# kspalaiologos/modern-rzip

Hardware: AMD Instinct MI355X
Metric: rzip-stage GiB/s (mrzip -n) (higher is better)
Workload: dtype u8; 1 GPU; tar-64G: rzip stage of mrzip -L7 on a 64 GiB synthetic tar (60 % text members, 25 % noise, 15 % exact duplicates, 512-byte aligned; BASELINE configs[2], the largest single-GPU configuration), one chunk per GPU, input resident in HBM; level=7, chunk_bytes_per_gpu=68719476736, streams=1, mode=streams

## Files before the change

### modern-rzip_amd/csrc/mrz_seq_deep.hip

```cpp
#ifndef MRZ_DEEP_WAVES
#define MRZ_DEEP_WAVES 8
#endif
#define MRZ_SEQ_WAVES MRZ_DEEP_WAVES
#include "mrz_seq_common.h"
#include <cstddef>

#ifndef MRZ_DEEP_LANES
#define MRZ_DEEP_LANES 256
#endif
#ifndef MRZ_DEEP_GROUP
#define MRZ_DEEP_GROUP 8
#endif
#define MRZ_DEEP_THREADS (64 * MRZ_DEEP_WAVES)
#ifdef __HIP_DEVICE_COMPILE__
#define MRZ_DEEP_WAIT() asm volatile("s_waitcnt vmcnt(0)" ::: "memory")
#else
#define MRZ_DEEP_WAIT() ((void)0)
#endif
#ifdef MRZ_SEQ_PROFILE
#define DPROF_T0() int64_t dprof_t0 = (int64_t)__builtin_amdgcn_s_memtime()
#define DPROF_T0R() dprof_t0 = (int64_t)__builtin_amdgcn_s_memtime()
#define DPROF_ADD(acc)                                               \
    do {                                                             \
        const int64_t now__ = (int64_t)__builtin_amdgcn_s_memtime(); \
// ... 100 lines not shown
    return (unsigned)fwd | (lngf << 7) | ((unsigned)rawb << 8);
}

__device__ __forceinline__ int mrz_deep_pair_eval(unsigned raw, int64_t q, int64_t op, int64_t floor_p) {
    if (op >= q) return 0;
    const int fwd = (int)(raw & 127u), rawb = (int)((raw >> 8) & 127u);
    int64_t maxb = q - floor_p;
    if (op < maxb) maxb = op;
    if (maxb < 0) maxb = 0;
    const int edge = op < 64 ? (int)(op >> 4) : 4;
    if (((raw >> 7) & 1u) || (rawb == 64 && maxb > 64) || (edge < 4 && rawb >= 16 * edge && maxb > 16 * edge)) return 1;
    const int rv = rawb < maxb ? rawb : (int)maxb;
    return fwd + rv >= MRZ_MIN_MATCH ? 1 : 0;
}

__device__ __forceinline__ unsigned mrz_deep_hs(unsigned x) { return (x * 2654435761u) >> (32 - 11); }
static_assert(MRZ_DEEP_MAP == 2048, "mrz_deep_hs gives 11 bits");
static_assert(MRZ_DEEP_LANES * 4 <= MRZ_DEEP_MAP * 3 / 4 || MRZ_DEEP_LANES <= 256, "the maps hold a batch's writes");

__device__ static void mrz_deep_smap_put(mrz_deep_lds *S, int slot, int lane_no) {
    const unsigned key = (unsigned)slot + 1u;
    unsigned i = mrz_deep_hs(key);
    for (int n = 0; n < MRZ_DEEP_MAP; n++) {
        const unsigned k = atomicCAS(&S->smap_key[i], 0u, key);
        if (k == 0u || k == key) {
            atomicMin(&S->smap_lane[i], lane_no);
            return;
        }
        i = (i + 1) & (MRZ_DEEP_MAP - 1);
    }
}
__device__ static int mrz_deep_smap_get(const mrz_deep_lds *S, int slot) {
    if (slot < 0) return 0x7fffffff;
    const unsigned key = (unsigned)slot + 1u;
    unsigned i = mrz_deep_hs(key);
    for (int n = 0; n < MRZ_DEEP_MAP; n++) {
        const unsigned k = S->smap_key[i];
        if (k == 0u) return 0x7fffffff;
        if (k == key) return S->smap_lane[i];
        i = (i + 1) & (MRZ_DEEP_MAP - 1);
    }
    return 0;
}
__device__ static void mrz_deep_tmap_put(mrz_deep_lds *S, int64_t tag, int lane_no) {
    if (tag == 0) return;
    const unsigned long long key = (unsigned long long)tag;
    unsigned i = mrz_deep_hs((unsigned)(key ^ (key >> 23)));
    for (int n = 0; n < MRZ_DEEP_MAP; n++) {
        const unsigned long long k = atomicCAS(&S->tmap_key[i], 0ull, key);
        if (k == 0ull || k == key) {
            atomicMin(&S->tmap_lane[i], lane_no);
            return;
        }
        i = (i + 1) & (MRZ_DEEP_MAP - 1);
    }
}
__device__ static int mrz_deep_tmap_get(const mrz_deep_lds *S, int64_t tag) {
    if (tag == 0) return 0x7fffffff;
    const unsigned long long key = (unsigned long long)tag;
    unsigned i = mrz_deep_hs((unsigned)(key ^ (key >> 23)));
    for (int n = 0; n < MRZ_DEEP_MAP; n++) {
        const unsigned long long k = S->tmap_key[i];
        if (k == 0ull) return 0x7fffffff;
        if (k == key) return S->tmap_lane[i];
        i = (i + 1) & (MRZ_DEEP_MAP - 1);
    }
    return 0;
}

__device__ __forceinline__ int mrz_deep_cw_slot(const mrz_deep_lds *S, int64_t cw_base, int r) {
    int lo = 0, hi = MRZ_DEEP_CW_WORDS - 1;
#pragma unroll
    for (int it = 0; it < 5; it++) {
        const int mid = (lo + hi + 1) >> 1;
        if (S->cwcum[mid] <= r)
            lo = mid;
        else
            hi = mid - 1;
    }
    return (int)(cw_base + lo * 64 + mrz_select64(S->cw[lo], r - S->cwcum[lo]));
}
static_assert(MRZ_DEEP_CW_WORDS == 32, "mrz_deep_cw_slot searches 32 words in 5 steps");

__device__ static void mrz_deep_scan(const mrz_cfg &C, mrz_deep_lds *S, int i, int64_t better, int64_t tag_mask,
                                     int64_t clean_ptr, int xw_n, int lane, int from = 0) {
    const mrz_slot *tab = C.tab;
    const uint8_t *__restrict__ buf = C.buf;
    const int smask = (int)C.slot_mask;
    const int max_chain = (int)C.max_chain;
    const int64_t q = mrz_uni64(S->R.q[i]), t = mrz_uni64(S->R.t[i]);
    const bool ins = (t & tag_mask) == tag_mask;
    const int my_rank = mrz_ones_rank(t);
    const int h = (int)(t & C.slot_mask);
    int fe = -1, w = -1, kind = ins ? -1 : MRZ_DK_NONE;
    int nsame = 0, round = 0;
    bool cplx = false;
    int64_t occ_t = 0, occ_off = 0, old_t = 0;
    bool cont = false, insert_kept = false, fe2 = false;
    int nsame0 = 0;
    int alt_w = -1, alt_kind = MRZ_DK_NONE, alt_st = 0, alt_round = 0;
    int64_t alt_old_t = 0;
    if (from > 0) {
        const int f0 = mrz_uni((int)S->R.flags[i]), k0 = mrz_uni((int)S->R.kind[i]);
        const int ns0 = mrz_uni((int)S->R.nsame[i]);
        if (!(f0 & MRZ_DF_CPLX) && k0 != MRZ_DK_EVICT && k0 != MRZ_DK_DISPLACE && from <= ((mrz_uni(S->R.fe[i]) - h) & smask)) {
            cont = true;
            const bool before = lane < ns0 && ((S->R.same_slot[i][lane < MRZ_SMAX ? lane : 0] - h) & smask) < from;
            nsame0 = nsame = __popcll(__ballot(before));
            if (ins && (k0 == MRZ_DK_EMPTY || k0 == MRZ_DK_OVER) && ((mrz_uni(S->R.w[i]) - h) & smask) < from) {
                insert_kept = true;
                kind = k0;
                w = mrz_uni(S->R.w[i]);
                old_t = mrz_uni64(S->R.old_t[i]);
            } else
                round = nsame;
        }
    }
    const int start = cont ? from : 0;
    const int max_groups = (int)((C.nslots + 64 * MRZ_DEEP_GROUP - 1) / (64 * MRZ_DEEP_GROUP)) + 1;
    for (int grp = 0; fe < 0; grp++) {
        if (grp >= max_groups) {
            cplx = true;
            fe = h;
            break;
        }
        mrz_slot e[MRZ_DEEP_GROUP];
        const int s0 = h + start + grp * (64 * MRZ_DEEP_GROUP) + lane;
#pragma unroll
        for (int g = 0; g < MRZ_DEEP_GROUP; g++) e[g] = tab[(s0 + g * 64) & smask];
#pragma unroll
        for (int g = 0; g < MRZ_DEEP_GROUP; g++) {
            if (fe >= 0) continue;
            const int sb = s0 - lane + g * 64;
            const bool empty = (e[g].off | e[g].t) == 0;
            const mrz_u64 m_empty = __ballot(empty);
            const int fe_idx = m_empty ? __ffsll((long long)m_empty) - 1 : 64;
            const mrz_u64 valid = mrz_low_mask(fe_idx);
            const mrz_u64 m_same = __ballot(!empty && e[g].t == t) & valid;
            mrz_u64 m_due = 0, m_low = 0;
            if (kind == -1 || alt_st == 1) {
                m_due = __ballot(!empty && (e[g].t & better) != better) & valid;
                m_low = __ballot(!empty && mrz_ones_rank(e[g].t) < my_rank) & valid & ~m_due;
            }
            int alt_from = 0;
            if (kind == -1) {
                const mrz_u64 m_stop = m_due | m_low;
                const int ks = m_stop ? __ffsll((long long)m_stop) - 1 : 64;
                const int nq = __popcll(m_same & mrz_low_mask(ks));
                if (round + nq >= max_chain) {
                    kind = MRZ_DK_EVICT;
                } else {
                    round += nq;
                    if (ks < 64) {
                        w = (sb + ks) & smask;
                        if ((m_due >> ks) & 1) {
                            kind = MRZ_DK_OVER;
                            old_t = mrz_bcast64(e[g].t, ks);
                            alt_st = 1;
                            alt_from = ks + 1;
                            alt_round = round;
                        } else {
                            kind = MRZ_DK_DISPLACE;
                            occ_t = mrz_bcast64(e[g].t, ks);
                            occ_off = mrz_bcast64(e[g].off, ks);
                        }
                    } else if (fe_idx < 64) {
                        w = (sb + fe_idx) & smask;
                        kind = MRZ_DK_EMPTY;
                        if (fe_idx < 63 && ((m_empty >> (fe_idx + 1)) & 1)) {
                            alt_w = (sb + fe_idx + 1) & smask;
                            alt_kind = MRZ_DK_EMPTY;
                        }
                        alt_st = 2;
                    }
                }
            }
            if (alt_st == 1 && alt_from < 64) {
                const mrz_u64 beyond = ~mrz_low_mask(alt_from);
                const mrz_u64 m_stop2 = (m_due | m_low) & beyond;
                const int ks2 = m_stop2 ? __ffsll((long long)m_stop2) - 1 : 64;
                const int nq2 = __popcll(m_same & beyond & mrz_low_mask(ks2));
                if (alt_round + nq2 >= max_chain)
                    alt_st = 2;
                else {
                    alt_round += nq2;
                    if (ks2 < 64) {
                        if ((m_due >> ks2) & 1) {
                            alt_w = (sb + ks2) & smask;
                            alt_kind = MRZ_DK_OVER;
                            alt_old_t = mrz_bcast64(e[g].t, ks2);
                        }
                        alt_st = 2;
                    } else if (fe_idx < 64) {
                        alt_w = (sb + fe_idx) & smask;
                        alt_kind = MRZ_DK_EMPTY;
                        alt_st = 2;
                    }
                }
            }
            if (m_same) {
                if ((m_same >> lane) & 1) {
                    const int k = nsame + __popcll(m_same & mrz_low_mask(lane));
                    if (k < MRZ_SMAX) {
                        S->R.same_slot[i][k] = (sb + lane) & smask;
                        S->R.same_off[i][k] = e[g].off;
                    }
                }
                nsame += __popcll(m_same);
            }
            if (fe_idx < 64) {
                fe = (sb + fe_idx) & smask;
                fe2 = fe_idx < 63 && ((m_empty >> (fe_idx + 1)) & 1);
            }
        }
    }
    if (nsame > MRZ_SMAX) cplx = true;
    if (kind == MRZ_DK_EVICT && max_chain > MRZ_SMAX) cplx = true;
    int h2 = 0, w2 = -1, kind2 = MRZ_DK_NONE;
    int64_t old_t2 = 0;
    if (kind == MRZ_DK_DISPLACE && !cplx) {
        const int rank2 = mrz_ones_rank(occ_t);
        h2 = (int)(occ_t & C.slot_mask);
        int round2 = 0;
        bool done = false;
        for (int grp = 0; !done; grp++) {
            if (grp >= max_groups) {
                cplx = true;
                break;
            }
            mrz_slot e[MRZ_DEEP_GROUP];
            const int s0 = h2 + grp * (64 * MRZ_DEEP_GROUP) + lane;
#pragma unroll
            for (int g = 0; g < MRZ_DEEP_GROUP; g++) e[g] = tab[(s0 + g * 64) & smask];
#pragma unroll
            for (int g = 0; g < MRZ_DEEP_GROUP; g++) {
                if (done) continue;
                const int sb = s0 - lane + g * 64;
                const bool empty = (e[g].off | e[g].t) == 0;
                const bool due = !empty && (e[g].t & better) != better;
                const bool low = !empty && !due && mrz_ones_rank(e[g].t) < rank2;
                const mrz_u64 m_empty = __ballot(empty), m_due = __ballot(due), m_low = __ballot(low);
                const mrz_u64 m_stop = m_empty | m_due | m_low;
                const int ks = m_stop ? __ffsll((long long)m_stop) - 1 : 64;
                const int nq = __popcll(__ballot(!empty && !due && !low && e[g].t == occ_t) & mrz_low_mask(ks));
                if (round2 + nq >= max_chain) {
                    cplx = true;
                    done = true;
                } else if (ks < 64) {
                    if ((m_low >> ks) & 1)
                        cplx = true;
                    else {
                        w2 = (sb + ks) & smask;
                        kind2 = ((m_empty >> ks) & 1) ? MRZ_DK_EMPTY : MRZ_DK_OVER;
                        if (kind2 == MRZ_DK_OVER) old_t2 = mrz_bcast64(e[g].t, ks);
                    }
                    done = true;
                } else
                    round2 += nq;
            }
        }
    }
    const int ns = nsame < MRZ_SMAX ? nsame : MRZ_SMAX;
    if (ns > nsame0) {
        MRZ_WAVE_SYNC();
        if (lane >= nsame0 && lane < ns) S->R.raw[i][lane] = (unsigned short)mrz_deep_probe_raw(buf, q, S->R.same_off[i][lane], C.end);
    }
    if (lane == 0) {
        S->R.h[i] = h;
        S->R.fe[i] = fe;
        S->R.w[i] = w;
        S->R.kind[i] = (unsigned char)(kind < 0 ? MRZ_DK_NONE : kind);
        S->R.h2[i] = h2;
        S->R.w2[i] = w2;
        S->R.kind2[i] = (unsigned char)kind2;
        S->R.occ_t[i] = occ_t;
        S->R.occ_off[i] = occ_off;
        S->R.old_t[i] = old_t;
        S->R.old_t2[i] = old_t2;
        S->R.alt_w[i] = (cplx || kind == MRZ_DK_DISPLACE || kind == MRZ_DK_EVICT || insert_kept) ? -1 : alt_w;
        S->R.alt_kind[i] = (unsigned char)alt_kind;
        S->R.alt_old_t[i] = alt_old_t;
        S->R.nsame[i] = (unsigned char)ns;
        S->R.flags[i] = (unsigned char)((ins ? MRZ_DF_INS : 0) | (cplx ? MRZ_DF_CPLX : 0) | (fe2 ? MRZ_DF_FE2 : 0));
        if (!cont) {
            S->R.cp_scan[i] = clean_ptr;
            S->R.xw_seen[i] = (unsigned short)xw_n;
        }
    }
}

#ifndef MRZ_DEEP_SCANNERS
#define MRZ_DEEP_SCANNERS 63
#endif
#define MRZ_DEEP_STAMP_RETRIES (1 << 20)
#ifndef MRZ_DEEP_HELP_MIN
#define MRZ_DEEP_HELP_MIN 48
#endif

#define MRZ_DEEP_REC_HDR 5
#define MRZ_DEEP_REC_GRANULES (MRZ_DEEP_REC_HDR + MRZ_SMAX)
struct mrz_deep_rec_ent {
    int64_t same_off;
    int same_slot;
    unsigned short raw, pad;
};
struct __attribute__((aligned(16))) mrz_deep_rec {
    int64_t occ_t, occ_off;
    int64_t old_t, old_t2;
    int64_t cp_scan, alt_old_t;
    int alt_w, h, fe, w;
    int h2, w2;
    unsigned short xw_seen;
    unsigned char kind, kind2, nsame, flags, alt_kind, pad;
    mrz_deep_rec_ent ent[MRZ_SMAX];
};
static_assert(sizeof(mrz_deep_rec_ent) == 16 && sizeof(mrz_deep_rec) == 16 * MRZ_DEEP_REC_GRANULES, "records travel as 16-byte granules");
// ... 102 lines not shown
#else
struct mrz_deep_recmem {
    char *base;
};
__device__ __forceinline__ mrz_deep_recmem mrz_deep_recmem_of(mrz_deep_shared *G) {
    mrz_deep_recmem m;
    m.base = (char *)G->rec;
    return m;
}
__device__ __forceinline__ void mrz_deep_granule_store(const mrz_deep_recmem &m, unsigned off, uint4 v) {
    *(uint4 *)(m.base + off) = v;
}
__device__ __forceinline__ uint4 mrz_deep_granule_load(const mrz_deep_recmem &m, bool take, unsigned off, int soff) {
    return take ? *(const uint4 *)(m.base + off + soff) : make_uint4(0, 0, 0, 0);
}
#endif

__device__ __forceinline__ void mrz_deep_rec_send(const mrz_deep_recmem &m, const mrz_deep_lds *S, int i, int lane) {
    MRZ_WAVE_SYNC();
    const int ng = MRZ_DEEP_REC_HDR + mrz_uni((int)S->R.nsame[i]);
    if (lane < ng) mrz_deep_granule_store(m, (unsigned)(i * (int)sizeof(mrz_deep_rec) + lane * 16), mrz_deep_rec_granule(&S->R, i, lane));
}

#define MRZ_DEEP_REC_FIRST (MRZ_DEEP_REC_HDR + 1)
#define MRZ_DEEP_FETCH_PER (MRZ_DEEP_THREADS / MRZ_DEEP_REC_FIRST)
__device__ __forceinline__ void mrz_deep_recs_fetch(mrz_deep_shared *G, mrz_deep_lds *S, int nb, int nscan, int tid) {
    const mrz_deep_recmem m = mrz_deep_recmem_of(G);
    constexpr int NLD = (MRZ_DEEP_LANES + MRZ_DEEP_FETCH_PER - 1) / MRZ_DEEP_FETCH_PER;
    constexpr int CH = 5;
#ifdef __HIP_DEVICE_COMPILE__
    asm volatile("" : "+v"(tid));
#endif
    const int i0 = tid / MRZ_DEEP_REC_FIRST, g = tid - i0 * MRZ_DEEP_REC_FIRST;
    const unsigned off0 = (unsigned)(i0 * (int)sizeof(mrz_deep_rec) + g * 16);
    bool take[NLD];
#pragma unroll
    for (int j = 0; j < NLD; j++) {
        const int i = i0 + j * MRZ_DEEP_FETCH_PER;
        take[j] = i0 < MRZ_DEEP_FETCH_PER && i < nb && i % nscan != 0;
    }
    uint4 v[NLD];
#pragma unroll
    for (int j = 0; j < NLD; j++) {
        v[j] = mrz_deep_granule_load(m, take[j], off0, j * MRZ_DEEP_FETCH_PER * (int)sizeof(mrz_deep_rec));
    }
#pragma unroll
    for (int j = 0; j < NLD; j++)
        if (take[j]) mrz_deep_rec_ungranule(&S->R, i0 + j * MRZ_DEEP_FETCH_PER, g, v[j], MRZ_SMAX);
    __syncthreads();
    const int ns = (tid < nb && tid % nscan != 0) ? (int)S->R.nsame[tid] : 0;
    for (int k0 = 1; __ballot(k0 < ns) != 0; k0 += CH) {
        const unsigned offe = (unsigned)(tid * (int)sizeof(mrz_deep_rec) + (MRZ_DEEP_REC_HDR + k0) * 16);
        uint4 e[CH];
#pragma unroll
        for (int c = 0; c < CH; c++) {
            e[c] = mrz_deep_granule_load(m, k0 + c < ns, offe, c * 16);
        }
#pragma unroll
        for (int c = 0; c < CH; c++)
            if (k0 + c < ns) mrz_deep_rec_ungranule(&S->R, tid, MRZ_DEEP_REC_HDR + k0 + c, e[c], ns);
    }
}

__device__ static void mrz_deep_scan_helper(const mrz_cfg &C, mrz_deep_lds *S, mrz_deep_shared *G, int tid, int lane, int wave) {
    if (tid == 0) {
        long long spins = 0;
        unsigned long long x = 0;
        while ((x = __hip_atomic_load(&G->xcc_plus1, __ATOMIC_RELAXED, __HIP_MEMORY_SCOPE_AGENT)) == 0 &&
               !__hip_atomic_load(&G->quit, __ATOMIC_RELAXED, __HIP_MEMORY_SCOPE_AGENT) && spins++ < (1ll << 24))
            __builtin_amdgcn_s_sleep(8);
        int ticket = -1;
        if (x != 0)
            ticket = (int)__hip_atomic_fetch_add(&G->n_ok, 1ull, __ATOMIC_RELAXED, __HIP_MEMORY_SCOPE_AGENT);
        S->ctl[0] = ticket;
    }
    __syncthreads();
    const int ticket = mrz_uni(S->ctl[0]);
    if (ticket < 0 || ticket >= MRZ_DEEP_SCANNERS) return;
    const int me = ticket + 1;
    const mrz_deep_recmem recmem = mrz_deep_recmem_of(G);
    unsigned long long seen = 0;
    int retries = 0;
#ifdef MRZ_SEQ_PROFILE
    int64_t hprof[4] = {0, 0, 0, 0};
#endif
    DPROF_T0();
    while (true) {
        if (tid == 0) {
            long long spins = 0;
            unsigned long long sq = 0;
            int v = 1;
            while (true) {
                sq = __hip_atomic_load(&G->seq, __ATOMIC_RELAXED, __HIP_MEMORY_SCOPE_AGENT);
                if (sq != seen && retries == 0) break;
                if (__hip_atomic_load(&G->quit, __ATOMIC_RELAXED, __HIP_MEMORY_SCOPE_AGENT) || spins++ > MRZ_HELPER_SPIN_LIMIT) {
                    v = 0;
                    break;
                }
                if (sq != seen) break;
                __builtin_amdgcn_s_sleep(2);
            }
            DPROF_T0R();
            MRZ_DEEP_ACQUIRE();
            MRZ_DEEP_WAIT();
            S->ctl[1] = v;
            S->lead.p = (int64_t)sq;
        }
        __syncthreads();
        if (!mrz_uni(S->ctl[1])) break;
        DPROF_ADD(hprof[0]);
        const unsigned long long sq = (unsigned long long)mrz_uni64(S->lead.p);
        const uint4 sv = *(const uint4 *)&G->stamp;
        const unsigned long long job_seq = (unsigned long long)mrz_uni64((int64_t)(((unsigned long long)sv.y << 32) | sv.x));
        const int nb = mrz_uni((int)sv.z), nscan = mrz_uni((int)sv.w);
        const int xw_n = (int)G->xw_n;
        const int64_t better = G->better, tag_mask = G->tag_mask, clean_ptr = G->clean_ptr;
        if (job_seq != sq) {
            if (++retries > MRZ_DEEP_STAMP_RETRIES) break;
            __syncthreads();
            continue;
        }
        retries = 0;
        seen = sq;
        int mine_n = 0;
        if (me < nscan) {
            for (int i = me + tid * nscan; i < nb; i += nscan * MRZ_DEEP_THREADS) {
                S->R.q[i] = G->q[i];
                S->R.t[i] = G->t[i];
            }
            __syncthreads();
            DPROF_ADD(hprof[1]);
            int k = 0;
            for (int i = me; i < nb; i += nscan, k++)
                if (k % MRZ_DEEP_WAVES == wave) {
                    mrz_deep_scan(C, S, i, better, tag_mask, clean_ptr, xw_n, lane);
                    mrz_deep_rec_send(recmem, S, i, lane);
                }
            mine_n = k;
            MRZ_DEEP_WAIT();
#ifdef MRZ_SEQ_PROFILE
            __syncthreads();
            DPROF_ADD(hprof[2]);
#endif
        }
        __syncthreads();
        if (tid == 0 && mine_n) {
#ifdef MRZ_DEEP_HANDOFF_FENCED
            MRZ_DEEP_RELEASE();
            MRZ_DEEP_WAIT();
#endif
            __hip_atomic_fetch_add(&G->done, (unsigned long long)mine_n, __ATOMIC_RELAXED, __HIP_MEMORY_SCOPE_AGENT);
            DPROF_ADD(hprof[3]);
        }
    }
#ifdef MRZ_SEQ_PROFILE
    if (tid == 0 && ticket == 0)
        for (int k = 0; k < 4; k++) C.st->prof[MRZ_ST_DH_T_ACQ + k] += hprof[k];
#endif
}

__device__ static __attribute__((noinline)) bool mrz_deep_coop(const mrz_cfg &C, mrz_lead &L, mrz_coop_lds *B, int64_t t,
                                                               int lane, int64_t *stat) {
    return mrz_seq_candidate(C, L, B, t, lane, stat);
}

__device__ static __attribute__((noinline)) bool mrz_deep_candidate_rec(const mrz_cfg &C, mrz_lead &L, mrz_deep_lds *S, int i, int *xw_n, int lane,
                                              int64_t *stat) {
    mrz_coop_lds *B = &S->coop;
    const int64_t q = mrz_uni64(S->R.q[i]), t = mrz_uni64(S->R.t[i]);
    const int ns = mrz_uni((int)S->R.nsame[i]);
    const int f = mrz_uni((int)S->R.flags[i]);
    int64_t mlen = 0, m_off = 0, m_rev = 0;
    L.p = q;
    if (ns) {
        if (lane < ns) {
            const int64_t op = S->R.same_off[i][lane];
            B->same_off[lane] = op;
            int64_t ml, rv;
            bool lng;
            mrz_lane_match_len(C.buf, q, op, C.end, L.last_match, &ml, &rv, &lng);
            B->pair_res[lane] = lng ? -1 : (int)((ml << 8) | rv);
        }
        MRZ_WAVE_SYNC();
        int xh = 0, xm = 0;
        if (!mrz_resolve_entries(C, L, B, q, ns, lane, stat, &mlen, &m_off, &m_rev, &xh, &xm)) return false;
        L.tag_hits += xh;
        L.tag_misses += xm;
    }
    int nx = *xw_n;
    if (f & MRZ_DF_INS) {
        const int kind = mrz_uni((int)S->R.kind[i]);
        L.inserts++;
        L.count++;
        int ws = mrz_uni(S->R.w[i]);
        if (kind == MRZ_DK_OVER)
            L.count--;
        else if (kind == MRZ_DK_EVICT) {
            L.count--;
            ws = mrz_uni(S->R.same_slot[i][(int)L.victim_round]);
            L.victim_round = L.victim_round + 1 == C.max_chain ? 0 : L.victim_round + 1;
        } else if (kind == MRZ_DK_DISPLACE) {
            const int w2 = mrz_uni(S->R.w2[i]);
            if (mrz_uni((int)S->R.kind2[i]) == MRZ_DK_OVER) L.count--;
            if (lane == 0) {
                mrz_slot oc;
                oc.off = S->R.occ_off[i];
                oc.t = S->R.occ_t[i];
                C.tab[w2] = oc;
                S->xw_slot[nx] = w2;
            }
            nx++;
        }
        if (lane == 0) {
            mrz_slot nw;
            nw.off = q;
            nw.t = t;
            C.tab[ws] = nw;
            S->xw_slot[nx] = ws;
        }
        nx++;
        if (L.count > C.limit) {
            MRZ_DEEP_WAIT();
            mrz_cull_one(C, L, lane);
            if (lane == 0) S->xw_slot[nx] = (int)L.clean_ptr;
            nx++;
        }
    }
    *xw_n = nx;
    return mrz_select_emit(C, L, mlen, m_off, m_rev, lane);
}

__device__ __forceinline__ int mrz_deep_incl(int v, int *ws, int lane, int wave, int *total) {
    const int incl = mrz_wave_incl_sum(v, lane);
    if (lane == 63) ws[wave] = incl;
    __syncthreads();
    int add = 0, tot = 0;
#pragma unroll
    for (int w = 0; w < MRZ_DEEP_WAVES; w++) {
        const int x = ws[w];
        tot += x;
// ... 603 lines not shown
                        ST_ADD(MRZ_ST_D_COOP, 1);
                        ST_ADD(MRZ_ST_D_COOP_REC, rec ? 1 : 0);
                        const bool same_masks = L.min_mask == mm0 && L.tag_mask == tm0;
                        const int nwr = rec ? 0 : mrz_uni(S->coop.n_written);
                        const int64_t cs = rec ? -1 : mrz_uni64(S->coop.cull_slot);
                        const bool room = nx + nwr + 1 <= MRZ_DEEP_XW;
                        if (rec)
                            nx = nx_rec;
                        else if (okc && same_masks && room && !loose) {
                            if (lane < nwr) S->xw_slot[nx + lane] = (int)S->coop.pend_h[lane];
                            nx += nwr;
                            if (cs >= 0) {
                                if (lane == 0) S->xw_slot[nx] = (int)cs;
                                nx++;
                            }
                        }
                        verdict = !okc ? 3 : ((same_masks && (room || loose) && L.p >= q) ? 1 : 2);
                        if (!(loose && verdict == 1)) break;
                        int j = cl + 1;
                        while (j < nb && mrz_uni64(S->R.q[j]) <= L.p) j++;
                        if (j >= nb) break;
                        cl = j;
                    }
                    if (lane == 0) {
                        S->lead = L;
                        S->ctl[0] = verdict;
                        S->ctl[5] = nx;
                    }
                    MRZ_DEEP_WAIT();
                }
                __syncthreads();
                L = S->lead;
                xw_n = mrz_uni(S->ctl[5]);
                const int v = mrz_uni(S->ctl[0]);
                if (v == 3) ok = false;
                if (v == 2) cut = true;
                {
                    const int i = tid;
                    const int nf = mrz_deep_first(i > coop_lane && i < nb && S->R.q[i] > L.p, S->wmin3, lane, wave, tid, nb);
                    next = nf;
                }
                PROF_ADD(MRZ_ST_D_T_COOP);
            }
        }
        if (ok) {
            if (cut || L.p > mrz_uni64(S->R.q[nb - 1])) {
                int64_t pos = L.p + 1;
                if (pos < K.seg_start) pos = K.seg_start;
                ci = mrz_cand_lower_bound(K, pos, lane);
            } else
                ci += n_examined;
        }
        __syncthreads();
    }
    if (ok && ci >= K.n && L.p < lim) L.p = lim;
#ifdef MRZ_SEQ_PROFILE
    stat[MRZ_ST_D_T_TOTAL] += (int64_t)__builtin_amdgcn_s_memtime() - launch_t0;
#endif
    if (tid == 0) {
        if (G) __hip_atomic_store(&G->quit, 1ull, __ATOMIC_RELAXED, __HIP_MEMORY_SCOPE_AGENT);
#if MRZ_HELPER_WGS > 0
        if (C.gmb) mrz_g_storeu(&C.gmb->quit, 1ull);
#endif
        st->p = L.p;
        st->cur_p = L.cur_p;
        st->cur_ofs = L.cur_ofs;
        st->cur_len = L.cur_len;
        st->last_match = L.last_match;
        st->min_mask = L.min_mask;
        st->tag_mask = L.tag_mask;
        st->count = L.count;
        st->clean_ptr = L.clean_ptr;
        st->victim_round = L.victim_round;
        st->n_events = L.n_events;
        st->inserts = L.inserts;
        st->tag_hits = L.tag_hits;
        st->tag_misses = L.tag_misses;
        st->finished = L.p >= C.end ? 1 : 0;
        st->hint_positions = L.p - hint_p0;
        st->hint_events = L.n_events - hint_ev0;
        st->hint_matched = L.mbytes;
#ifdef MRZ_SEQ_STATS
        for (int k = 0; k < MRZ_ST_N; k++)
            if (k < MRZ_ST_DH_T_ACQ || k > MRZ_ST_DH_T_OUT) st->prof[k] += stat[k];
#endif
    }
}

extern "C" hipError_t mrz_launch_sequencer_deep(hipStream_t stream, const uint8_t *buf, mrz_slot *tab, const mrz_cand *cand,
                                                const int *tile_off, const mrz_u64 *bitmap, mrz_event *events,
                                                mrz_seq_state *st, void *gmailbox, int n_helpers, int xcd, void *deep_shared,
                                                int scanners) {
    mrz_seq_args a;
    a.buf = buf;
    a.tab = tab;
    a.cand = cand;
    a.tile_off = tile_off;
    a.bitmap = bitmap;
    a.events = events;
    a.st = st;
    a.gmailbox = gmailbox;
    a.xcd = xcd & 7;
    a.deep_bits = 0;
#if MRZ_HELPER_WGS == 0
    n_helpers = 0;
#endif
    if (n_helpers > MRZ_HELPER_WGS) n_helpers = MRZ_HELPER_WGS;
    if (n_helpers < 0 || !gmailbox) n_helpers = 0;
    a.n_helpers = n_helpers;
    if (gmailbox) {
        hipError_t e = hipMemsetAsync(gmailbox, 0, sizeof(mrz_gmailbox), stream);
        if (e != hipSuccess) return e;
    }
    if (scanners < 0 || !deep_shared) scanners = 0;
    if (scanners > MRZ_DEEP_SCANNERS) scanners = MRZ_DEEP_SCANNERS;
    unsigned grid = (unsigned)(1 + a.n_helpers);
    if (grid < (unsigned)(a.xcd + 1)) grid = (unsigned)(a.xcd + 1);
#ifdef MRZ_EMU_LDS_PER_BLOCK
    if (scanners > 0) {
        grid = (unsigned)(8 * scanners + a.xcd + 1);
        emu::request_coresident();
    }
#else
    if (scanners > a.n_helpers / 2) scanners = a.n_helpers / 2;
    while (scanners > 0 && grid < (unsigned)(scanners + 2)) scanners--;
#endif
    if (deep_shared) {
        hipError_t e = hipMemsetAsync(deep_shared, 0, offsetof(mrz_deep_shared, q), stream);
        if (e != hipSuccess) return e;
    }
    hipLaunchKernelGGL(mrz_seq_deep_kernel, dim3(grid), dim3(MRZ_DEEP_THREADS), 0, stream, a, (mrz_deep_shared *)deep_shared,
                       scanners);
    return hipGetLastError();
}

extern "C" size_t mrz_seq_deep_shared_size(void) { return sizeof(mrz_deep_shared); }
```

### modern-rzip_amd/csrc/mrz_seq_stats.h

```cpp
#pragma once
#include "mrz_common.h"

#define MRZ_SEQ_STATS_LIST(X) \
    X(BATCHES, "batches") X(FORMED, "formed") X(COMMITTED, "committed") X(SEGMENTS, "segments") \
    X(EMITS, "emits") X(BACKJUMP, "backjump") X(REWALK, "rewalk") X(LONGRES, "longres") X(SEQ, "seq_cands") \
    X(CUT_CPLX, "cut_cplx") X(CUT_OVERFLOW, "cut_overflow") X(SKIPOUT, "skipout") X(CONF0, "conf0") \
    X(PAIRS, "pairs") X(T_FORM, "t_form") X(T_WALK, "t_walk") X(T_CONF, "t_conf") X(T_PAIRS, "t_pairs") \
    X(T_LOOP, "t_loop") X(T_REWALK, "t_rewalk") X(T_LONG, "t_long") X(T_SEQ, "t_seq") X(FARMED, "farmed") \
    X(L_POST, "l_post") X(L_STRIPE, "l_stripe") X(L_BWD, "l_bwd") X(L_WAIT, "l_wait") X(L_ROUNDS, "l_rounds") \
    X(F_POST, "f_post") X(F_WAIT, "f_wait") X(F_FOLD, "f_fold") X(S_TAB, "s_tab") X(S_PAIR, "s_pair") \
    X(S_INS, "s_ins") X(OVL, "ovl") X(OVL_OK, "ovl_ok") X(X_WALK, "x_walk") X(X_CASC, "x_casc") \
    X(X_POOL, "x_pool") X(X_WIN, "x_win") X(X_SAME, "x_same") X(C_WIN, "c_win") X(C_EVICT, "c_evict") \
    X(C_DEEP, "c_deep") X(C_MANY, "c_many") X(C_FAIL, "c_fail") X(C_TIE, "c_tie") X(C_NW, "c_nw") \
    X(T_OVL, "t_ovl") X(H_PRE, "h_pre") X(H_CAND, "h_cand") X(H_POST, "h_post") X(T_SCAN, "t_scan") \
    X(T_FOLD, "t_fold") X(T_COMMIT, "t_commit") X(REPREP, "reprep") X(W_STALE, "w_stale") X(W_DROP, "w_drop") \
    X(RESET, "reset") X(T_TURN, "t_turn") X(T_PREP, "t_prep") X(T_PRECOMMIT, "t_precommit") X(E_MASK, "e_mask") \
    X(E_CULL, "e_cull") X(E_XW, "e_xw") X(E_INWIN, "e_inwin") X(E_WINDOW, "e_window") X(E_BULK, "e_bulk") \
    X(E_MORE, "e_more") X(T_PC_CW, "t_pc_cw") X(T_PC_LOG, "t_pc_log") X(T_PC_BEST, "t_pc_best") \
    X(T_PC_BULK, "t_pc_bulk") X(T_TURNWORK, "t_turnwork") X(T_SNAP, "t_snap") X(REBULK, "rebulk") \
     \
    X(BATCH_LANES, "batch_lanes") X(CUT_LONG, "cut_long") X(CUT_WALK, "cut_walk") \
    X(CUT_CONFLICT, "cut_conflict") X(CUT_CULL, "cut_cull") X(BATCH_EMITS, "batch_emits") \
    X(CUT_CASCADE, "cut_cascade") X(BATCH_FORMED, "batch_formed") X(T_WALK2, "t_walk2") X(T_SCANS, "t_scans") \
    X(T_CONFLICT, "t_conflict") X(T_WINDOW, "t_window") \
     \
    X(D_BATCHES, "d_batches") X(D_LANES, "d_lanes") X(D_ROUNDS, "d_rounds") X(D_RESCANNED, "d_rescanned") \
    X(D_COOP, "d_coop") X(D_T_FORM, "d_t_form") X(D_T_SCAN, "d_t_scan") X(D_T_COMMIT, "d_t_commit") \
    X(D_T_RESCAN, "d_t_rescan") X(D_T_TOTAL, "d_t_total") X(D_LAUNCHES, "d_launches") X(D_T_COOP, "d_t_coop") \
    X(D_COOP_REC, "d_coop_rec") X(D_RESOLVED, "d_resolved") X(D_S_COOP, "d_s_coop") \
    X(D_S_CONFLICT, "d_s_conflict") X(D_S_CULLED, "d_s_culled") X(D_S_NOCULL, "d_s_nocull") \
    X(D_S_STALE, "d_s_stale") X(D_C_OVER_ALT, "d_c_over_alt") X(D_C_OVER_NOALT, "d_c_over_noalt") \
    X(D_C_EMPTY, "d_c_empty") X(D_C_DISPLACE, "d_c_displace") X(D_C_OTHER, "d_c_other") \
     \
    X(D_T_POST, "d_t_post") X(D_T_OWN, "d_t_own") X(D_T_WAIT, "d_t_wait") X(D_T_COPYIN, "d_t_copyin") \
    X(DH_T_ACQ, "dh_t_acq") X(DH_T_JOB, "dh_t_job") X(DH_T_SCAN, "dh_t_scan") X(DH_T_OUT, "dh_t_out")

#define MRZ_ST_ENUM(id, name) MRZ_ST_##id,
enum { MRZ_SEQ_STATS_LIST(MRZ_ST_ENUM) MRZ_ST_N };
#undef MRZ_ST_ENUM
static_assert(MRZ_ST_N <= (int)(sizeof(((mrz_seq_state *)0)->prof) / sizeof(int64_t)), "mrz_seq_state.prof holds the counters");
```

Baseline: 6.767 GiB/s.

## Double-buffer deep-scan table loads and skip quiet groups with one ballot

The deep hash-table scan now issues the next group of slot loads before processing the current one, using a two-set register buffer and a partial vmcnt wait, so memory latency overlaps the ballot logic. It also adds a fast path that skips a whole group when no lane sees an empty, same-tag or stop-worthy entry, replacing eight rounds of ballots with one. Scalar parameters are forced uniform and loads go through global address-space byte offsets to cut address arithmetic. The cost is more vector registers, which may lower occupancy, and one extra speculative group load per scan.

```diff
diff --git a/modern-rzip_amd/csrc/mrz_seq_deep.hip b/modern-rzip_amd/csrc/mrz_seq_deep.hip
--- a/modern-rzip_amd/csrc/mrz_seq_deep.hip
+++ b/modern-rzip_amd/csrc/mrz_seq_deep.hip
@@ -206,16 +206,70 @@
 }
 static_assert(MRZ_DEEP_CW_WORDS == 32, "mrz_deep_cw_slot searches 32 words in 5 steps");
 
+#if defined(__HIP_DEVICE_COMPILE__) && !defined(MRZ_DEEP_SCAN_FLAT)
+typedef long long mrz_deep_v2l __attribute__((ext_vector_type(2)));
+typedef const __attribute__((address_space(1))) char *mrz_deep_tab;
+__device__ __forceinline__ mrz_deep_tab mrz_deep_tab_of(const mrz_slot *tab) {
+    return (mrz_deep_tab)(uintptr_t)mrz_uni64((int64_t)(uintptr_t)tab);
+}
+__device__ __forceinline__ mrz_slot mrz_deep_tab_ld(mrz_deep_tab tab, unsigned byte_off) {
+    const mrz_deep_v2l v = *(const __attribute__((address_space(1))) mrz_deep_v2l *)(tab + byte_off);
+    mrz_slot e;
+    e.off = v.x;
+    e.t = v.y;
+    return e;
+}
+#else
+typedef const mrz_slot *mrz_deep_tab;
+__device__ __forceinline__ mrz_deep_tab mrz_deep_tab_of(const mrz_slot *tab) { return tab; }
+__device__ __forceinline__ mrz_slot mrz_deep_tab_ld(mrz_deep_tab tab, unsigned byte_off) { return tab[byte_off >> 4]; }
+#endif
+#if defined(__HIP_DEVICE_COMPILE__) && !defined(MRZ_DEEP_SCAN_VECTOR_STATE)
+#define MRZ_DEEP_UNI(v) mrz_uni(v)
+#define MRZ_DEEP_UNI64(v) mrz_uni64(v)
+#else
+#define MRZ_DEEP_UNI(v) (v)
+#define MRZ_DEEP_UNI64(v) (v)
+#endif
+#ifdef __HIP_DEVICE_COMPILE__
+#define MRZ_DEEP_SCHED_FENCE() __builtin_amdgcn_sched_barrier(0)
+#else
+#define MRZ_DEEP_SCHED_FENCE() ((void)0)
+#endif
+#ifdef MRZ_SEQ_PROFILE
+#define MRZ_DSCAN_PROF_PARAM , int64_t *wprof = nullptr
+#define DSCAN_T0() int64_t dscan_t0 = wprof ? (int64_t)__builtin_amdgcn_s_memtime() : 0
+#define DSCAN_WAIT(n) asm volatile("s_waitcnt vmcnt(%0) lgkmcnt(0)" ::"n"(n) : "memory")
+#define DSCAN_ADD(k)                                                     \
+    do {                                                                 \
+        if (wprof) {                                                     \
+            const int64_t now__ = (int64_t)__builtin_amdgcn_s_memtime(); \
+            wprof[k] += now__ - dscan_t0;                                \
+            dscan_t0 = now__;                                            \
+        }                                                                \
+    } while (0)
+#else
+#define MRZ_DSCAN_PROF_PARAM
+#define DSCAN_T0()
+#define DSCAN_WAIT(n)
+#define DSCAN_ADD(k)
+#endif
 __device__ static void mrz_deep_scan(const mrz_cfg &C, mrz_deep_lds *S, int i, int64_t better, int64_t tag_mask,
-                                     int64_t clean_ptr, int xw_n, int lane, int from = 0) {
-    const mrz_slot *tab = C.tab;
+                                     int64_t clean_ptr, int xw_n, int lane, int from = 0 MRZ_DSCAN_PROF_PARAM) {
+    i = MRZ_DEEP_UNI(i);
+    from = MRZ_DEEP_UNI(from);
+    xw_n = MRZ_DEEP_UNI(xw_n);
+    better = MRZ_DEEP_UNI64(better);
+    tag_mask = MRZ_DEEP_UNI64(tag_mask);
+    clean_ptr = MRZ_DEEP_UNI64(clean_ptr);
+    const mrz_deep_tab tab = mrz_deep_tab_of(C.tab);
     const uint8_t *__restrict__ buf = C.buf;
-    const int smask = (int)C.slot_mask;
-    const int max_chain = (int)C.max_chain;
+    const int smask = MRZ_DEEP_UNI((int)C.slot_mask);
+    const int max_chain = MRZ_DEEP_UNI((int)C.max_chain);
     const int64_t q = mrz_uni64(S->R.q[i]), t = mrz_uni64(S->R.t[i]);
     const bool ins = (t & tag_mask) == tag_mask;
     const int my_rank = mrz_ones_rank(t);
-    const int h = (int)(t & C.slot_mask);
+    const int h = (int)(t & (int64_t)smask);
     int fe = -1, w = -1, kind = ins ? -1 : MRZ_DK_NONE;
     int nsame = 0, round = 0;
     bool cplx = false;
@@ -241,110 +295,157 @@
         }
     }
     const int start = cont ? from : 0;
-    const int max_groups = (int)((C.nslots + 64 * MRZ_DEEP_GROUP - 1) / (64 * MRZ_DEEP_GROUP)) + 1;
-    for (int grp = 0; fe < 0; grp++) {
+    const int max_groups = (int)(((int64_t)smask + 1 + 64 * MRZ_DEEP_GROUP - 1) / (64 * MRZ_DEEP_GROUP)) + 1;
+    mrz_slot e2[2][MRZ_DEEP_GROUP];
+    const int sl = h + start + lane;
+    const unsigned bmask = (unsigned)smask << 4;
+    unsigned bo[MRZ_DEEP_GROUP];
+#pragma unroll
+    for (int g = 0; g < MRZ_DEEP_GROUP; g++) bo[g] = (((unsigned)sl << 4) + (unsigned)g * 1024u) & bmask;
+#define MRZ_DEEP_LOAD_NEXT_GROUP(set)                                                                          \
+    _Pragma("unroll") for (int g = 0; g < MRZ_DEEP_GROUP; g++) e2[set][g] = mrz_deep_tab_ld(tab, bo[g]);       \
+    MRZ_DEEP_SCHED_FENCE();                                                                                    \
+    _Pragma("unroll") for (int g = 0; g < MRZ_DEEP_GROUP; g++) bo[g] = (bo[g] + MRZ_DEEP_GROUP * 1024u) & bmask
+#ifndef MRZ_DEEP_SCAN_NO_AHEAD
+    MRZ_DEEP_LOAD_NEXT_GROUP(0);
+#endif
+#ifndef MRZ_DEEP_SCAN_NO_QUIET
+    const int64_t stop_bits = better | (int64_t)(my_rank > 0 ? mrz_low_mask(my_rank - 1) : 0ull);
+#endif
+    for (int grp = 0; fe < 0; grp += 2) {
         if (grp >= max_groups) {
             cplx = true;
             fe = h;
             break;
         }
-        mrz_slot e[MRZ_DEEP_GROUP];
-        const int s0 = h + start + grp * (64 * MRZ_DEEP_GROUP) + lane;
-#pragma unroll
-        for (int g = 0; g < MRZ_DEEP_GROUP; g++) e[g] = tab[(s0 + g * 64) & smask];
-#pragma unroll
-        for (int g = 0; g < MRZ_DEEP_GROUP; g++) {
+#pragma unroll
+        for (int half = 0; half < 2; half++) {
             if (fe >= 0) continue;
-            const int sb = s0 - lane + g * 64;
-            const bool empty = (e[g].off | e[g].t) == 0;
-            const mrz_u64 m_empty = __ballot(empty);
-            const int fe_idx = m_empty ? __ffsll((long long)m_empty) - 1 : 64;
-            const mrz_u64 valid = mrz_low_mask(fe_idx);
-            const mrz_u64 m_same = __ballot(!empty && e[g].t == t) & valid;
-            mrz_u64 m_due = 0, m_low = 0;
-            if (kind == -1 || alt_st == 1) {
-                m_due = __ballot(!empty && (e[g].t & better) != better) & valid;
-                m_low = __ballot(!empty && mrz_ones_rank(e[g].t) < my_rank) & valid & ~m_due;
+            const int gi = grp + half;
+            DSCAN_T0();
+#ifdef MRZ_DEEP_SCAN_NO_AHEAD
+            MRZ_DEEP_LOAD_NEXT_GROUP(half);
+            DSCAN_WAIT(0);
+#else
+            MRZ_DEEP_LOAD_NEXT_GROUP(half ^ 1);
+            MRZ_DEEP_SCHED_FENCE();
+            DSCAN_WAIT(MRZ_DEEP_GROUP);
+#endif
+            DSCAN_ADD(0);
+            const mrz_slot(&e)[MRZ_DEEP_GROUP] = e2[half];
+            const int s0 = h + start + gi * (64 * MRZ_DEEP_GROUP);
+#ifndef MRZ_DEEP_SCAN_NO_QUIET
+            {
+                const bool open = kind == -1 || alt_st == 1;
+                bool loud = false;
+#pragma unroll
+                for (int g = 0; g < MRZ_DEEP_GROUP; g++) {
+                    const int64_t et = e[g].t;
+                    loud |= ((e[g].off | et) == 0) | (et == t);
+                    if (open) loud |= ((et & stop_bits) != stop_bits) | (et == -1);
+                }
+                if (__ballot(loud) == 0 && (kind != -1 || round < max_chain) && (alt_st != 1 || alt_round < max_chain)) {
+                    DSCAN_ADD(1);
+                    continue;
+                }
             }
-            int alt_from = 0;
-            if (kind == -1) {
-                const mrz_u64 m_stop = m_due | m_low;
-                const int ks = m_stop ? __ffsll((long long)m_stop) - 1 : 64;
-                const int nq = __popcll(m_same & mrz_low_mask(ks));
-                if (round + nq >= max_chain) {
-                    kind = MRZ_DK_EVICT;
-                } else {
-                    round += nq;
-                    if (ks < 64) {
-                        w = (sb + ks) & smask;
-                        if ((m_due >> ks) & 1) {
-                            kind = MRZ_DK_OVER;
-                            old_t = mrz_bcast64(e[g].t, ks);
-                            alt_st = 1;
-                            alt_from = ks + 1;
-                            alt_round = round;
-                        } else {
-                            kind = MRZ_DK_DISPLACE;
-                            occ_t = mrz_bcast64(e[g].t, ks);
-                            occ_off = mrz_bcast64(e[g].off, ks);
-                        }
-                    } else if (fe_idx < 64) {
-                        w = (sb + fe_idx) & smask;
-                        kind = MRZ_DK_EMPTY;
-                        if (fe_idx < 63 && ((m_empty >> (fe_idx + 1)) & 1)) {
-                            alt_w = (sb + fe_idx + 1) & smask;
+#endif
+#pragma unroll
+            for (int g = 0; g < MRZ_DEEP_GROUP; g++) {
+                if (fe >= 0) continue;
+                const int sb = s0 + g * 64;
+                const bool empty = (e[g].off | e[g].t) == 0;
+                const mrz_u64 m_empty = __ballot(empty);
+                const int fe_idx = m_empty ? __ffsll((long long)m_empty) - 1 : 64;
+                const mrz_u64 valid = mrz_low_mask(fe_idx);
+                const mrz_u64 m_same = __ballot(!empty && e[g].t == t) & valid;
+                mrz_u64 m_due = 0, m_low = 0;
+                if (kind == -1 || alt_st == 1) {
+                    m_due = __ballot(!empty && (e[g].t & better) != better) & valid;
+                    m_low = __ballot(!empty && mrz_ones_rank(e[g].t) < my_rank) & valid & ~m_due;
+                }
+                int alt_from = 0;
+                if (kind == -1) {
+                    const mrz_u64 m_stop = m_due | m_low;
+                    const int ks = m_stop ? __ffsll((long long)m_stop) - 1 : 64;
+                    const int nq = __popcll(m_same & mrz_low_mask(ks));
+                    if (round + nq >= max_chain) {
+                        kind = MRZ_DK_EVICT;
+                    } else {
+                        round += nq;
+                        if (ks < 64) {
+                            w = (sb + ks) & smask;
+                            if ((m_due >> ks) & 1) {
+                                kind = MRZ_DK_OVER;
+                                old_t = mrz_bcast64(e[g].t, ks);
+                                alt_st = 1;
+                                alt_from = ks + 1;
+                                alt_round = round;
+                            } else {
+                                kind = MRZ_DK_DISPLACE;
+                                occ_t = mrz_bcast64(e[g].t, ks);
+                                occ_off = mrz_bcast64(e[g].off, ks);
+                            }
+                        } else if (fe_idx < 64) {
+                            w = (sb + fe_idx) & smask;
+                            kind = MRZ_DK_EMPTY;
+                            if (fe_idx < 63 && ((m_empty >> (fe_idx + 1)) & 1)) {
+                                alt_w = (sb + fe_idx + 1) & smask;
+                                alt_kind = MRZ_DK_EMPTY;
+                            }
+                            alt_st = 2;
+                        }
+                    }
+                }
+                if (alt_st == 1 && alt_from < 64) {
+                    const mrz_u64 beyond = ~mrz_low_mask(alt_from);
+                    const mrz_u64 m_stop2 = (m_due | m_low) & beyond;
+                    const int ks2 = m_stop2 ? __ffsll((long long)m_stop2) - 1 : 64;
+                    const int nq2 = __popcll(m_same & beyond & mrz_low_mask(ks2));
+                    if (alt_round + nq2 >= max_chain)
+                        alt_st = 2;
+                    else {
+                        alt_round += nq2;
+                        if (ks2 < 64) {
+                            if ((m_due >> ks2) & 1) {
+                                alt_w = (sb + ks2) & smask;
+                                alt_kind = MRZ_DK_OVER;
+                                alt_old_t = mrz_bcast64(e[g].t, ks2);
+                            }
+                            alt_st = 2;
+                        } else if (fe_idx < 64) {
+                            alt_w = (sb + fe_idx) & smask;
                             alt_kind = MRZ_DK_EMPTY;
-                        }
-                        alt_st = 2;
+                            alt_st = 2;
+                        }
                     }
                 }
+                if (m_same) {
+                    if ((m_same >> lane) & 1) {
+                        const int k = nsame + __popcll(m_same & mrz_low_mask(lane));
+                        if (k < MRZ_SMAX) {
+                            S->R.same_slot[i][k] = (sb + lane) & smask;
+                            S->R.same_off[i][k] = e[g].off;
+                        }
+                    }
+                    nsame += __popcll(m_same);
+                }
+                if (fe_idx < 64) {
+                    fe = (sb + fe_idx) & smask;
+                    fe2 = fe_idx < 63 && ((m_empty >> (fe_idx + 1)) & 1);
+                }
             }
-            if (alt_st == 1 && alt_from < 64) {
-                const mrz_u64 beyond = ~mrz_low_mask(alt_from);
-                const mrz_u64 m_stop2 = (m_due | m_low) & beyond;
-                const int ks2 = m_stop2 ? __ffsll((long long)m_stop2) - 1 : 64;
-                const int nq2 = __popcll(m_same & beyond & mrz_low_mask(ks2));
-                if (alt_round + nq2 >= max_chain)
-                    alt_st = 2;
-                else {
-                    alt_round += nq2;
-                    if (ks2 < 64) {
-                        if ((m_due >> ks2) & 1) {
-                            alt_w = (sb + ks2) & smask;
-                            alt_kind = MRZ_DK_OVER;
-                            alt_old_t = mrz_bcast64(e[g].t, ks2);
-                        }
-                        alt_st = 2;
-                    } else if (fe_idx < 64) {
-                        alt_w = (sb + fe_idx) & smask;
-                        alt_kind = MRZ_DK_EMPTY;
-                        alt_st = 2;
-                    }
-                }
-            }
-            if (m_same) {
-                if ((m_same >> lane) & 1) {
-                    const int k = nsame + __popcll(m_same & mrz_low_mask(lane));
-                    if (k < MRZ_SMAX) {
-                        S->R.same_slot[i][k] = (sb + lane) & smask;
-                        S->R.same_off[i][k] = e[g].off;
-                    }
-                }
-                nsame += __popcll(m_same);
-            }
-            if (fe_idx < 64) {
-                fe = (sb + fe_idx) & smask;
-                fe2 = fe_idx < 63 && ((m_empty >> (fe_idx + 1)) & 1);
-            }
-        }
-    }
+            DSCAN_ADD(1);
+        }
+    }
+#undef MRZ_DEEP_LOAD_NEXT_GROUP
     if (nsame > MRZ_SMAX) cplx = true;
     if (kind == MRZ_DK_EVICT && max_chain > MRZ_SMAX) cplx = true;
     int h2 = 0, w2 = -1, kind2 = MRZ_DK_NONE;
     int64_t old_t2 = 0;
     if (kind == MRZ_DK_DISPLACE && !cplx) {
         const int rank2 = mrz_ones_rank(occ_t);
-        h2 = (int)(occ_t & C.slot_mask);
+        h2 = (int)(occ_t & (int64_t)smask);
         int round2 = 0;
         bool done = false;
         for (int grp = 0; !done; grp++) {
@@ -355,7 +456,7 @@
             mrz_slot e[MRZ_DEEP_GROUP];
             const int s0 = h2 + grp * (64 * MRZ_DEEP_GROUP) + lane;
 #pragma unroll
-            for (int g = 0; g < MRZ_DEEP_GROUP; g++) e[g] = tab[(s0 + g * 64) & smask];
+            for (int g = 0; g < MRZ_DEEP_GROUP; g++) e[g] = mrz_deep_tab_ld(tab, (unsigned)((s0 + g * 64) & smask) << 4);
 #pragma unroll
             for (int g = 0; g < MRZ_DEEP_GROUP; g++) {
                 if (done) continue;
@@ -624,7 +725,7 @@
     unsigned long long seen = 0;
     int retries = 0;
 #ifdef MRZ_SEQ_PROFILE
-    int64_t hprof[4] = {0, 0, 0, 0};
+    int64_t hprof[6] = {0, 0, 0, 0, 0, 0};
 #endif
     DPROF_T0();
     while (true) {
@@ -675,7 +776,11 @@
             int k = 0;
             for (int i = me; i < nb; i += nscan, k++)
                 if (k % MRZ_DEEP_WAVES == wave) {
+#ifdef MRZ_SEQ_PROFILE
+                    mrz_deep_scan(C, S, i, better, tag_mask, clean_ptr, xw_n, lane, 0, ticket == 0 && wave == 0 ? &hprof[4] : nullptr);
+#else
                     mrz_deep_scan(C, S, i, better, tag_mask, clean_ptr, xw_n, lane);
+#endif
                     mrz_deep_rec_send(recmem, S, i, lane);
                 }
             mine_n = k;
@@ -697,7 +802,7 @@
     }
 #ifdef MRZ_SEQ_PROFILE
     if (tid == 0 && ticket == 0)
-        for (int k = 0; k < 4; k++) C.st->prof[MRZ_ST_DH_T_ACQ + k] += hprof[k];
+        for (int k = 0; k < 6; k++) C.st->prof[MRZ_ST_DH_T_ACQ + k] += hprof[k];
 #endif
 }
 
@@ -1467,7 +1572,7 @@
         st->hint_matched = L.mbytes;
 #ifdef MRZ_SEQ_STATS
         for (int k = 0; k < MRZ_ST_N; k++)
-            if (k < MRZ_ST_DH_T_ACQ || k > MRZ_ST_DH_T_OUT) st->prof[k] += stat[k];
+            if (k < MRZ_ST_DH_T_ACQ || k > MRZ_ST_DH_T_FOLD) st->prof[k] += stat[k];
 #endif
     }
 }
diff --git a/modern-rzip_amd/csrc/mrz_seq_stats.h b/modern-rzip_amd/csrc/mrz_seq_stats.h
--- a/modern-rzip_amd/csrc/mrz_seq_stats.h
+++ b/modern-rzip_amd/csrc/mrz_seq_stats.h
@@ -33,7 +33,8 @@
     X(D_C_EMPTY, "d_c_empty") X(D_C_DISPLACE, "d_c_displace") X(D_C_OTHER, "d_c_other") \
      \
     X(D_T_POST, "d_t_post") X(D_T_OWN, "d_t_own") X(D_T_WAIT, "d_t_wait") X(D_T_COPYIN, "d_t_copyin") \
-    X(DH_T_ACQ, "dh_t_acq") X(DH_T_JOB, "dh_t_job") X(DH_T_SCAN, "dh_t_scan") X(DH_T_OUT, "dh_t_out")
+    X(DH_T_ACQ, "dh_t_acq") X(DH_T_JOB, "dh_t_job") X(DH_T_SCAN, "dh_t_scan") X(DH_T_OUT, "dh_t_out") \
+    X(DH_T_LDWAIT, "dh_t_ldwait") X(DH_T_FOLD, "dh_t_fold")
 
 #define MRZ_ST_ENUM(id, name) MRZ_ST_##id,
 enum { MRZ_SEQ_STATS_LIST(MRZ_ST_ENUM) MRZ_ST_N };
```

Result: faster. 7.055 GiB/s, median of 6 (+4.2%).
